# secastel/phaser

Hardware: AMD Instinct MI355X
Metric: het-SNP allele calls/sec + phased variants/sec, whole-genome RNA-seq, 1→8 GPUs (higher is better)
Workload: dtype u8/int32; 1 GPU; configs[2]: whole genome (22 autosomes), one GTEx-shape RNA-seq sample, 79999998 records x 76 bp, 1499988 het SNPs, one shard per chromosome; chromosomes LPT-assigned to GPUs by record count; records=79999998, het_snps=1499988

## Files before the change

### phaser_amd/csrc/phz_map.hip

```cpp
#include "phz_internal.h"
#include "phz_lbound.h"
#include "phz_stagepack.h"
#include <stdlib.h>
#include <string.h>

namespace {

#ifndef PHZ_MAP_WIN
#define PHZ_MAP_WIN 512
#endif
#ifndef PHZ_CIG_X2
#define PHZ_CIG_X2 5
#endif
#ifndef PHZ_CAND_X4
#define PHZ_CAND_X4 3
#endif
constexpr int MAP_WIN = PHZ_MAP_WIN;

constexpr uint32_t OP_M = 0, OP_I = 1, OP_D = 2, OP_N = 3, OP_S = 4, OP_EQ = 7, OP_X = 8, OP_G = 9;

struct MapArgs {
    const int32_t *pos;
    const uint32_t *cigar_off, *cigar, *seq_off;
    const uint8_t *seq2, *qual;
    const uint8_t *bq;
    int64_t n;
    const int32_t *vpos;
    int nv;
    int baseq;
    uint2 *stage;
    uint32_t *side;
    int64_t slots;
    const int32_t *tile_w0;
    int32_t *tile_total;
    int slot_cap;
    int64_t ntiles;
    int dbg;
    bool one;
    const struct ShardDev *shp;
};

struct ShardDev {
    const int32_t *pos;
    const uint32_t *cigar_off, *cigar, *seq_off;
    const uint8_t *seq2, *qual;
    const uint8_t *bq;
    int64_t n;
    const int32_t *vpos;
    int nv, pad;
    int32_t *o_read, *o_var;
    uint8_t *o_code;
    uint32_t *o_aux0, *o_aux1;
    int64_t cap;
};

struct MapBatch {
    const ShardDev *shards;
    const int64_t *tile0;
    int n_shards, baseq;
    uint2 *stage;
    uint32_t *side; int64_t slots;
    int32_t *tile_w0;
    int32_t *tile_total;
    int slot_cap, dbg;
    int64_t ntiles;
    unsigned long long *prof;
    const struct OvfArea *ovf;
};
struct OvfArea { uint32_t *tile_first; unsigned long long *cursor; long long base, cap; };

__device__ __forceinline__ int shard_of(const int64_t *tile0, int n_shards, int64_t T) {
    int lo = 0, hi = n_shards - 1;
    while (lo < hi) {
        const int m = (lo + hi + 1) >> 1;
        if (tile0[m] <= T) lo = m; else hi = m - 1;
    }
    return lo;
}

__device__ __noinline__ int masked_base_escape(const MapArgs &a, uint32_t soff, int x) {
    const uint8_t *qual = a.shp->qual, *seq2 = a.shp->seq2;
    const uint32_t q = qual[(size_t)soff * 4 + x], s = (seq2[(size_t)soff + (x >> 2)] >> (2 * (x & 3))) & 3;
    if ((int)(q & 0x7f) < a.baseq) return 4;
    if (q & 0x80) return s == 0 ? 4 : 5;
    return (int)s;
}

struct VarWin {
    const int32_t *g;
    const int32_t *lds;
    int w0, nv, wlen;
    __device__ __forceinline__ int at(int i) const {
        unsigned d = (unsigned)(i - w0);
        return d < (unsigned)wlen ? lds[d] : g[i];
    }
    __device__ __forceinline__ int lower_bound(int lo, int key) const {
        int hi = nv;
        if (lo >= hi) return hi;
        int step = 1;
        while (lo + step < hi && at(lo + step) < key) { lo += step; step <<= 1; }
        if (lo < hi && at(lo) >= key) return lo;
        int h = lo + step < hi ? lo + step : hi;
        int l = lo + 1;
        while (l < h) {
            int m = (l + h) >> 1;
            if (at(m) < key) l = m + 1; else h = m;
        }
        return l;
    }
};

__device__ __forceinline__ void stage_put(uint2 *stage, uint32_t *side, int64_t slots, int64_t g, uint32_t var, uint32_t a0, uint32_t a1,
                                          uint32_t rec, uint32_t code) {
    const bool w0 = a0 >= 0x10000u, w1 = a1 != 0u;
    stage[g] = make_uint2(var, rec | (code << 10) | ((uint32_t)w1 << 14) | ((uint32_t)w0 << 15) | (w0 ? 0u : a0 << 16));
    if (w0) side[g] = a0;
    if (w1) side[slots + g] = a1;
}

struct CigWin {
    const uint32_t *g;
    const uint32_t *lds;
    uint32_t c_begin, cap;
    __device__ __forceinline__ uint32_t at(uint32_t k) const {
        const uint32_t d = k - c_begin;
        return d < cap ? lds[d] : g[k];
    }
};

#ifndef PHZ_CAND_INS
#define PHZ_CAND_INS 16
#endif
constexpr int CAND_INS = PHZ_CAND_INS;
constexpr uint32_t KEY_HAS_INS = 0x4000u;
struct CandBuf {
    uint32_t *key;
    uint16_t *var;
    uint16_t *x0;
    unsigned long long *ins;
    int *n;
    int *nins;
    int cap, w0;
};
__device__ __forceinline__ void cand_put(const CandBuf &cb, int slot, uint32_t key, int var, uint32_t x0, uint32_t x1) {
    const uint32_t dv = (uint32_t)(var - cb.w0);
    bool wide = dv >= 0xFFFFu || (x0 != 0xFFFFFFFFu && x0 >= 0xFFFFu);
    if (x1 != 0u) {
        const int t = atomicAdd(cb.nins, 1);
        if (t < CAND_INS) cb.ins[t] = ((unsigned long long)(uint32_t)slot << 32) | x1; else wide = true;
        key |= KEY_HAS_INS;
    }
    if (wide) atomicOr(cb.n, 1 << 30);
    cb.key[slot] = key;
    cb.var[slot] = (uint16_t)dv;
    cb.x0[slot] = (uint16_t)(x0 == 0xFFFFFFFFu ? 0xFFFFu : x0);
}
__device__ __forceinline__ uint32_t cand_x0(const CandBuf &cb, int e) { const uint32_t v = cb.x0[e]; return v == 0xFFFFu ? 0xFFFFFFFFu : v; }
__device__ __forceinline__ uint32_t cand_x1(const CandBuf &cb, int e, uint32_t key) {
    if (!(key & KEY_HAS_INS)) return 0u;
    const int m = *cb.nins < CAND_INS ? *cb.nins : CAND_INS;
    for (int t = 0; t < m; t++) { const unsigned long long w = cb.ins[t]; if ((int)(w >> 32) == e) return (uint32_t)w; }
    return 0u;
}

#define PHZ_SEQ_BYTE(a, soff, x) (((a).dbg & 1024) ? (a).qual[(size_t)(soff) * 4 + ((x) | 3)] : (a).seq2[(size_t)(soff) + ((x) >> 2)])
#define PHZ_ONEPLANE(a) ((a).one)
__device__ __forceinline__ int masked_base_two(const MapArgs &a, uint32_t soff, int x) {
    const uint32_t q = a.qual[(size_t)soff * 4 + x], s = (a.seq2[(size_t)soff + (x >> 2)] >> (2 * (x & 3))) & 3;
    if ((int)(q & 0x7f) < a.baseq) return 4;
    if (q & 0x80) return s == 0 ? 4 : 5;
    return (int)s;
}
__device__ int masked_base_escape(const MapArgs &a, uint32_t soff, int x);
__device__ __forceinline__ int sym_from_bq(const MapArgs &a, uint32_t soff, int x, uint32_t b) {
    const uint32_t q6 = b & 63u;
    if (q6 == 63u) return a.qual ? masked_base_two(a, soff, x) : masked_base_escape(a, soff, x);
    return (int)q6 < a.baseq ? 4 : (int)(b >> 6);
}
__device__ __forceinline__ int masked_base(const MapArgs &a, uint32_t soff, int x) {
    if (PHZ_ONEPLANE(a)) return sym_from_bq(a, soff, x, a.bq[(size_t)soff * 4 + x]);
    uint32_t q = a.qual[(size_t)soff * 4 + x];
    uint32_t s = (PHZ_SEQ_BYTE(a, soff, x) >> (2 * (x & 3))) & 3;
    if ((int)(q & 0x7f) < a.baseq) return 4;
    if (q & 0x80) return s == 0 ? 4 : 5;
    return (int)s;
}

template <int MODE, bool NARROW = false>
__device__ int walk_read(const MapArgs &a, const VarWin &vw, const CigWin &cw, const CandBuf &cb, int j, int64_t r, int pos,
                         uint32_t c0, uint32_t c1, uint32_t soff, int64_t out_base, int64_t out_limit) {
    int i = vw.lower_bound(vw.w0, pos);
    if (i >= vw.nv) return 0;
    int cnt = 0;
    int gpos = 0, rpos = 0, seg_start = 0, plen = 0, seg_rpos = 0;
    uint32_t seg_op = c0;
    for (uint32_t k = c0; k < c1; k++) {
        uint32_t w = cw.at(k);
        const int len = (int)(w >> 4);
        const uint32_t op = w & 15;
        if (op == OP_M || op == OP_EQ || op == OP_X || op == OP_D) {
            const int lo = pos + seg_start + plen, hi = lo + len;
            if (i < vw.nv && vw.at(i) < lo) i = vw.lower_bound(i, lo);
            while (i < vw.nv && !(a.dbg & 16)) {
                const int vp = vw.at(i);
                if (vp >= hi) break;
                const int p = vp - pos - seg_start;
                const int rb = rpos + (p - plen);
                int ioff = 0, ilen = 0;
                if (c1 - c0 > 1) {
                    int g2 = seg_start, r2 = seg_rpos;
                    for (uint32_t k2 = seg_op; k2 < c1; k2++) {
                        uint32_t w2 = cw.at(k2);
                        const int l2 = (int)(w2 >> 4);
                        const uint32_t o2 = w2 & 15;
                        if (o2 == OP_N) break;
                        if (o2 == OP_M || o2 == OP_EQ || o2 == OP_X) { g2 += l2; r2 += l2; }
                        else if (o2 == OP_D || o2 == OP_G) g2 += l2;
                        else if (o2 == OP_I) { if (g2 - 1 == p) { ioff = r2; ilen = l2; } r2 += l2; }
                        else if (o2 == OP_S) r2 += l2;
                    }
                }
                const int nchars = (op != OP_D) + ilen;
                if (nchars > 0) {
                    const uint32_t x0 = op != OP_D ? (uint32_t)rb : 0xFFFFFFFFu;
                    const uint32_t x1 = ilen > 0 ? (((uint32_t)ioff << 12) | (uint32_t)(ilen > 4095 ? 4095 : ilen)) : 0u;
                    if (MODE == 0) {
                        const int slot = cnt < 32 ? atomicAdd(cb.n, 1) : (atomicOr(cb.n, 1 << 30), 1 << 30);
                        if (slot < cb.cap) cand_put(cb, slot, ((uint32_t)j << 16) | ((uint32_t)cnt << 8) | (nchars == 1 ? 7u : 4u), i, x0, x1);
                        cnt++;
                    } else {
                        int code = 4;
                        if (nchars == 1) {
                            const int s = masked_base(a, soff, op != OP_D ? rb : ioff);
                            code = s < 4 ? s : (s == 4 ? -1 : 4);
                        }
                        if (code >= 0) {
                            if (MODE == 2) {
                                const int64_t o = out_base + cnt;
                                if (o < out_limit) {
                                    if (NARROW) reinterpret_cast<uint32_t *>(a.stage)[o] = stage4_pack((uint32_t)i, (uint32_t)j, (uint32_t)code);
                                    else stage_put(a.stage, a.side, a.slots, o, (uint32_t)i, x0, x1, (uint32_t)j, (uint32_t)code);
                                }
                            }
                            cnt++;
                        }
                    }
                }
                i++;
            }
            plen += len; gpos += len;
            if (op != OP_D) rpos += len;
        } else if (op == OP_I || op == OP_S) {
            rpos += len;
        } else if (op == OP_N) {
            gpos += len; seg_start = gpos; plen = 0; seg_op = k + 1; seg_rpos = rpos;
        } else if (op == OP_G) {
            gpos += len;
        }
    }
    return cnt;
}

#ifndef PHZ_WIN_DSMALL
#define PHZ_WIN_DSMALL 7
#endif
constexpr int WIN_DMAX = 31 - __builtin_clz((unsigned)MAP_WIN);
constexpr int WIN_DSMALL = WIN_DMAX < PHZ_WIN_DSMALL ? WIN_DMAX : PHZ_WIN_DSMALL;
static_assert(MAP_WIN >= 2 && MAP_WIN <= 1024 && (MAP_WIN & (MAP_WIN - 1)) == 0, "MAP_WIN: a power of two up to 1024");
__device__ __forceinline__ int window_depth(int wlen) {
    return wlen <= (1 << WIN_DSMALL) ? WIN_DSMALL : WIN_DMAX;
}
__device__ __forceinline__ int lds_lower_bound(const int32_t *w, int wdepth, int key) {
    return wdepth == WIN_DSMALL ? window_lower_bound<WIN_DSMALL>(w, key) : window_lower_bound<WIN_DMAX>(w, key);
}

__device__ bool walk_lean(const int32_t *s_vpos, int wlen, int wdepth, int w0, const uint32_t *s_cig, uint32_t c_begin, uint32_t cig_cap,
                          const CandBuf &cb, uint32_t *s_poison, int j, int pos, uint32_t c0, uint32_t c1, long long cover, int dbg) {
    if (c1 - c_begin > cig_cap) return false;
    int g = 0, seg_start = 0, cnt = 0, nins = 0; uint32_t r = 0;
    bool bad = false;
    int t0 = -1, t1 = -1; uint32_t o0 = 0, o1 = 0, l0 = 0, l1 = 0;
    uint32_t prev = 0x10u, prev_len = 1;
    for (uint32_t k = c0; k < c1; k++) {
        const uint32_t w = s_cig[k - c_begin];
        const int len = (int)(w >> 4); const uint32_t op = w & 15, bit = 1u << op;
        const bool mlike = (bit & 0x181u) != 0;
        if (__builtin_amdgcn_uicmp(op, OP_I, 32 ) != 0) {
            if (op == OP_I) {
                bad |= (prev & 0x272u) != 0 || prev_len == 0 || nins == 2;
                nins++;
                t1 = t0; o1 = o0; l1 = l0; t0 = g - 1 + seg_start; o0 = r; l0 = (uint32_t)(len > 4095 ? 4095 : len);
            }
        }
        bad |= op == OP_G;
        const bool search = (mlike || op == OP_D) && !(dbg & 64);
        if (__builtin_amdgcn_ballot_w64(search) != 0) {
            const int lo = pos + g;
            bad |= search && (long long)lo + len > cover;
            const int hi = (search && !bad) ? lo + len : lo;
            int i = lds_lower_bound(s_vpos, wdepth, lo);
            while (i < wlen && !(dbg & 128)) {
                const int vp = s_vpos[i];
                if (vp >= hi) break;
                uint32_t ioff = 0, ilen = 0;
                if (seg_start == 0) {
                    if (vp == hi - 1 && k + 1 < c1) {
                        const uint32_t wn = s_cig[k + 1 - c_begin];
                        if ((wn & 15) == OP_I) { ilen = wn >> 4; ilen = ilen > 4095u ? 4095u : ilen; ioff = r + (mlike ? (uint32_t)len : 0u); }
                    }
                } else {
                    const int off = vp - pos;
                    if (t0 == off) { ioff = o0; ilen = l0; } else if (t1 == off) { ioff = o1; ilen = l1; }
                }
                const int nchars = (mlike ? 1 : 0) + (int)ilen;
                if (nchars > 0) {
                    const int slot = cnt < 32 ? atomicAdd(cb.n, 1) : (atomicOr(cb.n, 1 << 30), 1 << 30);
                    if (slot < cb.cap)
                        cand_put(cb, slot, ((uint32_t)j << 16) | ((uint32_t)(cnt | 0x80) << 8) | (nchars == 1 ? 7u : 4u), w0 + i,
                                 mlike ? (uint32_t)(r + (uint32_t)(vp - lo)) : 0xFFFFFFFFu, ilen > 0 ? ((ioff << 12) | ilen) : 0u);
                    cnt++;
                }
                i++;
            }
        }
        g += len & __builtin_amdgcn_sbfe(0x38D, op, 1u);
        r += (uint32_t)(len & __builtin_amdgcn_sbfe(0x193, op, 1u));
        if (op == OP_N) { seg_start = g; t0 = -1; t1 = -1; }
        prev = bit; prev_len = (uint32_t)len;
    }
    if (bad) atomicOr(&s_poison[j >> 5], 1u << (j & 31));
    return !bad;
}

constexpr int MAP_COVER = 65536;
constexpr int MAP_SLACK = 8;

__global__ void k_tile_window(MapBatch bt, int tile_reads) {
    const int64_t T = (int64_t)blockIdx.x * blockDim.x + threadIdx.x;
    if (T == 0) *bt.ovf->cursor = 0ull;
    const bool live = T < bt.ntiles;
    const int si = live ? shard_of(bt.tile0, bt.n_shards, T) : 0;
    const ShardDev &sh = bt.shards[si];
    const int64_t t = live ? T - bt.tile0[si] : 0;
    const int32_t *pos = sh.pos; const uint32_t *cigar_off = sh.cigar_off; const int32_t *vpos = sh.vpos;
    const int nv = sh.nv; const int64_t n = sh.n;
    int32_t *tile_w = bt.tile_w0;
    const int key = live ? pos[t * tile_reads] : 0;
    const uint32_t coff0 = live ? cigar_off[t * tile_reads] : 0u;
    const int nb_key = __shfl_down(key, 1);
    const uint32_t nb_coff0 = (uint32_t)__shfl_down((int)coff0, 1);
    if (!live) return;
    const bool more = (t + 1) * tile_reads < n;
    const int64_t last = more ? (t + 1) * tile_reads - 1 : n - 1;
    const bool nb = more && (threadIdx.x & 63) != 63;
    const uint32_t coff_end = nb ? nb_coff0 : cigar_off[last + 1];
    const int pos_end = (nb && (long long)nb_key - key <= MAP_COVER) ? nb_key : pos[last];
    const long long key2 = (long long)pos_end + MAP_COVER;
    int lo = 0, hi = nv, lo2 = 0, hi2 = nv;
    while (lo < hi || lo2 < hi2) {
        const int m = (lo + hi) >> 1, m2 = (lo2 + hi2) >> 1;
        const bool go = lo < hi, go2 = lo2 < hi2;
        const int v = go ? vpos[m] : 0, v2 = go2 ? vpos[m2] : 0;
        if (go) { if (v < key) lo = m + 1; else hi = m; }
        if (go2) { if ((long long)v2 < key2) lo2 = m2 + 1; else hi2 = m2; }
    }
    int len = lo2 - lo + MAP_SLACK;
    int complete = 1 << 30;
    if (len > MAP_WIN) { len = MAP_WIN; complete = 0; }
    const uint32_t n_ops = coff_end - coff0;
    tile_w[4 * T] = lo;
    tile_w[4 * T + 1] = len | complete | (si << 16);
    tile_w[4 * T + 2] = (int32_t)coff0;
    tile_w[4 * T + 3] = (int32_t)n_ops;
}

__device__ __forceinline__ int wave_incl_scan(int v0) {
    int v1 = v0 + __builtin_amdgcn_update_dpp(0, v0, 0x111, 0xf, 0xf, true);
    v1 += __builtin_amdgcn_update_dpp(0, v0, 0x112, 0xf, 0xf, true);
    v1 += __builtin_amdgcn_update_dpp(0, v0, 0x113, 0xf, 0xf, true);
    v1 += __builtin_amdgcn_update_dpp(0, v1, 0x114, 0xf, 0xe, true);
    v1 += __builtin_amdgcn_update_dpp(0, v1, 0x118, 0xf, 0xc, true);
    v1 += __builtin_amdgcn_update_dpp(0, v1, 0x142, 0xa, 0xf, true);
    v1 += __builtin_amdgcn_update_dpp(0, v1, 0x143, 0xc, 0xf, true);
    return v1;
}

__device__ __forceinline__ int wave_max(int v0) {
    const int lo = (int)0x80000000;
    auto mx = [](int a, int b) { return a > b ? a : b; };
    int v1 = mx(v0, __builtin_amdgcn_update_dpp(lo, v0, 0x111, 0xf, 0xf, false));
    v1 = mx(v1, __builtin_amdgcn_update_dpp(lo, v0, 0x112, 0xf, 0xf, false));
    v1 = mx(v1, __builtin_amdgcn_update_dpp(lo, v0, 0x113, 0xf, 0xf, false));
    v1 = mx(v1, __builtin_amdgcn_update_dpp(lo, v1, 0x114, 0xf, 0xe, false));
    v1 = mx(v1, __builtin_amdgcn_update_dpp(lo, v1, 0x118, 0xf, 0xc, false));
    v1 = mx(v1, __builtin_amdgcn_update_dpp(lo, v1, 0x142, 0xa, 0xf, false));
    v1 = mx(v1, __builtin_amdgcn_update_dpp(lo, v1, 0x143, 0xc, 0xf, false));
    return __builtin_amdgcn_readlane(v1, 63);
}

template <int MAP_BLOCK, int RPT>
__device__ __forceinline__ int block_scan(const int (&cnt)[RPT], int (&excl)[RPT], int (*s_wsum)[MAP_BLOCK / 64], int lane, int wave) {
    int incl[RPT];
#pragma unroll
    for (int k = 0; k < RPT; k++) {
        const int x = wave_incl_scan(cnt[k]);
        incl[k] = x;
        if (lane == 63) s_wsum[k][wave] = x;
    }
    __syncthreads();
    int running = 0;
#pragma unroll
    for (int k = 0; k < RPT; k++) {
        int before = running;
#pragma unroll
        for (int w2 = 0; w2 < MAP_BLOCK / 64; w2++) {
            const int s = s_wsum[k][w2];
            if (w2 < wave) before += s;
            running += s;
        }
        excl[k] = before + incl[k] - cnt[k];
    }
    return running;
}

template <int MAP_BLOCK, int RPT, bool ABL, bool ONE, bool NARROW>
__device__ __forceinline__ void map_tile(const MapBatch &bt, const int64_t gtile) {
    const int4 tw = *reinterpret_cast<const int4 *>(bt.tile_w0 + 4 * gtile);
    const int si = (tw.y >> 16) & 0x1FFF;
    MapArgs a;
    {
        const ShardDev &sh = bt.shards[si];
        a.pos = sh.pos; a.cigar_off = sh.cigar_off; a.cigar = sh.cigar; a.seq_off = sh.seq_off; a.bq = sh.bq; a.shp = &sh;
        if (ONE && !ABL) { a.seq2 = nullptr; a.qual = nullptr; } else { a.seq2 = sh.seq2; a.qual = sh.qual; }
        a.n = sh.n; a.vpos = sh.vpos; a.nv = sh.nv; a.baseq = bt.baseq;
        a.stage = bt.stage; a.side = bt.side; a.slots = bt.slots;
        a.tile_w0 = bt.tile_w0; a.tile_total = bt.tile_total; a.slot_cap = bt.slot_cap; a.ntiles = bt.ntiles; a.dbg = ABL ? bt.dbg : 0;
        a.one = ABL ? ((bt.dbg & 4096) != 0 && sh.bq != nullptr) : ONE;
    }
#define PHZ_STAMP(K) do { if (ABL && (bt.dbg & 2048) && threadIdx.x == 0) bt.prof[8 * gtile + (K)] = wall_clock64(); } while (0)
    PHZ_STAMP(0);
    constexpr int TILE = MAP_BLOCK * RPT;
    constexpr int CIG = TILE * PHZ_CIG_X2 / 2;
    constexpr int CAND = TILE * PHZ_CAND_X4 / 4;
    __shared__ int32_t s_vpos[MAP_WIN];
    __shared__ uint32_t s_coff[TILE + 1];
    __shared__ uint32_t s_soff[TILE];
    __shared__ int32_t s_pos[TILE];
    uint32_t *s_mask = reinterpret_cast<uint32_t *>(s_pos);
    __shared__ uint16_t s_cx[TILE];
    __shared__ uint32_t s_cig[CIG];
    __shared__ uint32_t s_key[CAND];
    __shared__ uint16_t s_var[CAND];
    __shared__ uint16_t s_x0[CAND];
    __shared__ unsigned long long s_ins[CAND_INS];
    __shared__ int s_wsum[RPT][MAP_BLOCK / 64];
    __shared__ int s_ncand, s_ncx, s_nlong, s_nins;
    __shared__ uint32_t s_poison[TILE / 32];

    const int tid = threadIdx.x, lane = tid & 63, wave = tid >> 6;
    const int64_t tile = gtile - bt.tile0[si];
    const int64_t r0 = tile * TILE;
    const int nr = (int)((a.n - r0) < TILE ? (a.n - r0) : TILE);

    VarWin vw;
    vw.g = a.vpos; vw.lds = s_vpos; vw.nv = a.nv; vw.w0 = tw.x;
    vw.wlen = tw.y & 0xFFFF;
    const bool complete = (tw.y >> 30) & 1;
    CigWin cw;
    cw.g = a.cigar; cw.lds = s_cig; cw.c_begin = (uint32_t)tw.z; cw.cap = CIG;
    uint32_t cnt_w = (uint32_t)tw.w;
    if (cnt_w > (uint32_t)CIG) cnt_w = CIG;
    int rpos_[RPT];
    uint32_t soff_[RPT], coff_[RPT];
#pragma unroll
    for (int k = 0; k < RPT; k++) {
        const int j = k * MAP_BLOCK + tid;
        const bool ok = j < nr;
        rpos_[k] = ok ? a.pos[r0 + j] : 0;
        soff_[k] = ok ? a.seq_off[r0 + j] : 0;
        coff_[k] = a.cigar_off[r0 + (ok ? j : nr)];
    }
    const uint32_t coff_end = a.cigar_off[r0 + nr];
    int v_first = 0x7fffffff;
    if (tid < vw.wlen) { const int idx = vw.w0 + tid; v_first = idx < a.nv ? a.vpos[idx] : 0x7fffffff; }
    uint32_t cg[3] = {0, 0, 0};
#pragma unroll
    for (int u = 0; u < 3; u++) { const uint32_t j = (uint32_t)tid + (uint32_t)u * MAP_BLOCK; if (j < cnt_w) cg[u] = a.cigar[cw.c_begin + j]; }
#pragma unroll
    for (int k = 0; k < RPT; k++) {
        const int j = k * MAP_BLOCK + tid;
        s_pos[j] = rpos_[k]; s_soff[j] = soff_[k]; s_coff[j] = coff_[k];
    }
    if (tid == 0) { s_coff[TILE] = coff_end; s_ncand = 0; s_ncx = 0; s_nlong = 0; s_nins = 0; }
    if (tid < TILE / 32) s_poison[tid] = 0;
    const int wdepth = window_depth(vw.wlen);
#ifdef PHZ_FILL_ALL
    const int wfill = MAP_WIN;
#else
    const int wfill = (1 << wdepth) > vw.wlen ? (1 << wdepth) : vw.wlen;
#endif
    if (tid < wfill) s_vpos[tid] = v_first;
    for (int j = tid + MAP_BLOCK; j < wfill; j += MAP_BLOCK) {
        const int idx = vw.w0 + j;
        s_vpos[j] = (j < vw.wlen && idx < a.nv) ? a.vpos[idx] : 0x7fffffff;
    }
#pragma unroll
    for (int u = 0; u < 3; u++) { const uint32_t j = (uint32_t)tid + (uint32_t)u * MAP_BLOCK; if (j < cnt_w) s_cig[j] = cg[u]; }
    for (uint32_t j = (uint32_t)tid + 3u * MAP_BLOCK; j < cnt_w; j += MAP_BLOCK) s_cig[j] = a.cigar[cw.c_begin + j];
    __syncthreads();
    PHZ_STAMP(1);
    CandBuf cb;
    cb.key = s_key; cb.var = s_var; cb.x0 = s_x0; cb.ins = s_ins; cb.n = &s_ncand; cb.nins = &s_nins; cb.cap = CAND; cb.w0 = vw.w0;
    const long long cover = (long long)s_pos[nr - 1] + MAP_COVER;

    uint32_t c0_[RPT], c1_[RPT];
    int base_[RPT], n_[RPT];
    uint32_t vmask_[RPT], codes_[RPT];
    bool fast_[RPT];
#pragma unroll
    for (int k = 0; k < RPT; k++) {
        const int j = k * MAP_BLOCK + tid;
        c0_[k] = s_coff[j]; c1_[k] = s_coff[j + 1];
        base_[k] = 0; n_[k] = 0; vmask_[k] = 0; codes_[k] = 0; fast_[k] = false;
    }
    const bool walk_on = !(a.dbg & 8);
    int len_[RPT]; bool one_[RPT];
#pragma unroll
    for (int k = 0; k < RPT; k++) {
        const int j = k * MAP_BLOCK + tid;
        one_[k] = false; len_[k] = 0;
        const uint32_t d = c0_[k] - cw.c_begin;
        if (j < nr && walk_on && complete && c1_[k] - c0_[k] == 1 && d < (uint32_t)CIG) {
            const uint32_t w = s_cig[d];
            const uint32_t op = w & 15;
            len_[k] = (int)(w >> 4);
            one_[k] = (op == OP_M || op == OP_EQ || op == OP_X) && (long long)rpos_[k] + len_[k] <= cover;
        }
    }
    constexpr int GROUP = 64 / (2 * RPT);
    int target = 0x7fffffff;
#pragma unroll
    for (int k = 0; k < RPT; k++) {
        const int e = wave_max(one_[k] ? rpos_[k] + len_[k] : (int)0x80000000);
        const int first = __builtin_amdgcn_readfirstlane(rpos_[k]);
        if ((lane / GROUP) == 2 * k) target = first;
        if ((lane / GROUP) == 2 * k + 1) target = e;
    }
    const int bound = lds_lower_bound(s_vpos, wdepth, target);
#pragma unroll
    for (int k = 0; k < RPT; k++) {
        const int j = k * MAP_BLOCK + tid;
        const int lo = __builtin_amdgcn_readlane(bound, 2 * k * GROUP), hi = __builtin_amdgcn_readlane(bound, (2 * k + 1) * GROUP);
        if (one_[k]) {
            const int pos = rpos_[k], end = pos + len_[k];
            if (hi - lo <= 24) {
                int below = 0, c = 0;
                for (int e = lo; e < hi; e++) {
                    const int vp = s_vpos[e];
                    below += vp < pos ? 1 : 0;
                    c += (vp >= pos && vp < end) ? 1 : 0;
                }
                if (c <= 8) { fast_[k] = true; base_[k] = lo + below; n_[k] = c; }
            } else {
                const int base = lds_lower_bound(s_vpos, wdepth, pos);
                int c = 0;
                while (base + c < vw.wlen && s_vpos[base + c] < end && c <= 8) c++;
                if (c <= 8) { fast_[k] = true; base_[k] = base; n_[k] = c; }
            }
        }
        if (j < nr && walk_on && !fast_[k]) {
            if (s_coff[j + 1] - s_coff[j] > 3u) s_cx[TILE - 1 - atomicAdd(&s_nlong, 1)] = (uint16_t)j;
            else s_cx[atomicAdd(&s_ncx, 1)] = (uint16_t)j;
        }
    }
    uint32_t pre_q[RPT], pre_s[RPT];
#pragma unroll
    for (int k = 0; k < RPT; k++) {
        pre_q[k] = 0; pre_s[k] = 0;
        if (fast_[k] && n_[k] > 0 && !(a.dbg & 1)) {
            const uint32_t soff = s_soff[k * MAP_BLOCK + tid];
            const int x = s_vpos[base_[k]] - rpos_[k];
            if (PHZ_ONEPLANE(a)) pre_q[k] = a.bq[(size_t)soff * 4 + x];
            else { pre_q[k] = a.qual[(size_t)soff * 4 + x]; pre_s[k] = PHZ_SEQ_BYTE(a, soff, x); }
        }
    }
    PHZ_STAMP(2);
    __syncthreads();
    PHZ_STAMP(3);
    const int nshort = walk_on ? s_ncx : 0;
    const int ncx = (walk_on && !(a.dbg & 256)) ? nshort + s_nlong : 0;
    const bool lean_on = complete && !(a.dbg & 32);
    bool redo_any = false;
    for (int t = tid; t < ncx; t += MAP_BLOCK) {
        const int ts = t < nshort ? t : TILE - 1 - (t - nshort);
        const int j = s_cx[ts];
        const bool done = lean_on && walk_lean(s_vpos, vw.wlen, wdepth, vw.w0, s_cig, cw.c_begin, (uint32_t)CIG, cb, s_poison, j, s_pos[j], s_coff[j], s_coff[j + 1], cover, a.dbg);
        if (!done) { s_cx[ts] = (uint16_t)(j | 0x8000); redo_any = true; }
    }
    const bool redo = __syncthreads_or(redo_any ? 1 : 0) != 0;
#pragma unroll
    for (int k = 0; k < RPT; k++) s_mask[k * MAP_BLOCK + tid] = 0;
    if (redo) {
        for (int t = tid; t < ncx; t += MAP_BLOCK) {
            const int jf = s_cx[t < nshort ? t : TILE - 1 - (t - nshort)];
            if (jf & 0x8000) { const int j = jf & 0x7FFF; walk_read<0>(a, vw, cw, cb, j, r0 + j, a.pos[r0 + j], s_coff[j], s_coff[j + 1], 0, 0, 0); }
        }
    }
    __syncthreads();
    PHZ_STAMP(4);
    const int ncand = s_ncand;
    const bool fb = ncand > CAND;
    uint32_t cq = 0, cs = 0; int cx_off = -1;
    if (!fb && tid < ncand && !(a.dbg & 1)) {
        const uint32_t key = s_key[tid];
        if ((key & 0xFF) == 7u) {
            const uint32_t x0 = cand_x0(cb, tid);
            cx_off = x0 != 0xFFFFFFFFu ? (int)x0 : (int)(cand_x1(cb, tid, key) >> 12);
            const uint32_t soff = s_soff[key >> 16];
            if (PHZ_ONEPLANE(a)) cq = a.bq[(size_t)soff * 4 + cx_off];
            else { cq = a.qual[(size_t)soff * 4 + cx_off]; cs = PHZ_SEQ_BYTE(a, soff, cx_off); }
        }
    }
#pragma unroll
    for (int k = 0; k < RPT; k++) {
        if (!fast_[k]) continue;
        const int j = k * MAP_BLOCK + tid;
        const uint32_t soff = s_soff[j];
        for (int o = 0; o < n_[k]; o++) {
            const int x = s_vpos[base_[k] + o] - rpos_[k];
            int sy;
            if (a.dbg & 1) sy = x & 3;
            else if (o == 0) {
                if (PHZ_ONEPLANE(a)) sy = sym_from_bq(a, soff, x, pre_q[k]);
                else {
                    const uint32_t q = pre_q[k], sb = (pre_s[k] >> (2 * (x & 3))) & 3;
                    sy = (int)(q & 0x7f) < a.baseq ? 4 : ((q & 0x80) ? (sb == 0 ? 4 : 5) : (int)sb);
                }
            } else sy = masked_base(a, soff, x);
            if (sy != 4) { vmask_[k] |= 1u << o; codes_[k] |= (uint32_t)(sy < 4 ? sy : 4) << (4 * o); }
        }
    }
    int cnt[RPT], off[RPT];
    if (!fb) {
        for (int e = tid; e < ncand; e += MAP_BLOCK) {
            uint32_t key = s_key[e];
            const int j = (int)(key >> 16);
            int code = (int)(key & 0xFF);
            if ((key & 0x8000u) && ((s_poison[j >> 5] >> (j & 31)) & 1u)) code = -1;
            else if (code == 7) {
                const uint32_t x0 = cand_x0(cb, e);
                const int x = x0 != 0xFFFFFFFFu ? (int)x0 : (int)(cand_x1(cb, e, key) >> 12);
                int sy;
                if (a.dbg & 1) sy = x & 3;
                else if (e == tid && cx_off == x) {
                    if (PHZ_ONEPLANE(a)) sy = sym_from_bq(a, s_soff[j], x, cq);
                    else {
                        const uint32_t sb = (cs >> (2 * (x & 3))) & 3;
                        sy = (int)(cq & 0x7f) < a.baseq ? 4 : ((cq & 0x80) ? (sb == 0 ? 4 : 5) : (int)sb);
                    }
                } else sy = masked_base(a, s_soff[j], x);
                code = sy < 4 ? sy : (sy == 4 ? -1 : 4);
            }
            if (code >= 0) {
                atomicOr(&s_mask[j], 1u << ((key >> 8) & 31));
                s_key[e] = (key & 0xFFFFFF00u) | (uint32_t)code;
            } else {
                s_key[e] = key | 0xFFu;
            }
        }
        __syncthreads();
#pragma unroll
        for (int k = 0; k < RPT; k++) cnt[k] = fast_[k] ? __popc(vmask_[k]) : __popc(s_mask[k * MAP_BLOCK + tid]);
    } else {
#pragma unroll
        for (int k = 0; k < RPT; k++) {
            const int j = k * MAP_BLOCK + tid;
            cnt[k] = fast_[k] ? __popc(vmask_[k])
                              : (j < nr && walk_on ? walk_read<1>(a, vw, cw, cb, j, r0 + j, NARROW ? a.pos[r0 + j] : rpos_[k], NARROW ? s_coff[j] : c0_[k],
                                                                  NARROW ? s_coff[j + 1] : c1_[k], s_soff[j], 0, 0) : 0);
        }
    }
    PHZ_STAMP(5);
    const int T = block_scan<MAP_BLOCK, RPT>(cnt, off, s_wsum, lane, wave);
#pragma unroll
    for (int k = 0; k < RPT; k++) s_coff[k * MAP_BLOCK + tid] = (uint32_t)off[k];
    if (tid == 0) {
        a.tile_total[gtile] = T;
        uint32_t first = (uint32_t)(gtile * (int64_t)a.slot_cap);
        int room = a.slot_cap;
        if (T > a.slot_cap) {
            const OvfArea ov = *bt.ovf;
            const unsigned long long at = atomicAdd(ov.cursor, (unsigned long long)T);
            const bool fits = at + (unsigned long long)T <= (unsigned long long)ov.cap;
            if (fits) { first = (uint32_t)(ov.base + (long long)at); room = T; }
            ov.tile_first[gtile] = fits ? first : 0xFFFFFFFFu;
        }
        s_ncx = (int)first; s_nlong = room;
    }
    __syncthreads();
    PHZ_STAMP(6);
    if (a.dbg & 2) return;
    const int64_t slot0 = (int64_t)(uint32_t)s_ncx;
    const int slot_n = s_nlong;
#pragma unroll
    for (int k = 0; k < RPT; k++) {
        const int j = k * MAP_BLOCK + tid;
        if (fast_[k]) {
            int o2 = off[k];
            for (int o = 0; o < n_[k]; o++) {
                if (!((vmask_[k] >> o) & 1)) continue;
                if (o2 < slot_n) {
                    const int64_t g = slot0 + o2;
                    if (NARROW) reinterpret_cast<uint32_t *>(a.stage)[g] = stage4_pack((uint32_t)(vw.w0 + base_[k] + o), (uint32_t)j, (codes_[k] >> (4 * o)) & 15u);
                    else stage_put(a.stage, a.side, a.slots, g, (uint32_t)(vw.w0 + base_[k] + o), (uint32_t)(s_vpos[base_[k] + o] - rpos_[k]), 0u,
                                   (uint32_t)j, (codes_[k] >> (4 * o)) & 15u);
                }
                o2++;
            }
        } else if (fb && cnt[k] > 0) {
            walk_read<2, NARROW>(a, vw, cw, cb, j, r0 + j, NARROW ? a.pos[r0 + j] : rpos_[k], NARROW ? a.cigar_off[r0 + j] : c0_[k],
                                 NARROW ? a.cigar_off[r0 + j + 1] : c1_[k], s_soff[j], slot0 + off[k], slot0 + slot_n);
        }
    }
    if (!fb) {
        for (int e = tid; e < ncand; e += MAP_BLOCK) {
            const uint32_t key = s_key[e];
            if ((key & 0xFF) == 0xFF) continue;
            const int j = (int)(key >> 16);
            const uint32_t ord = (key >> 8) & 31;
            const int o = (int)s_coff[j] + __popc(s_mask[j] & ((1u << ord) - 1));
            if (o < slot_n) {
                const int64_t g = slot0 + o;
                if (NARROW) reinterpret_cast<uint32_t *>(a.stage)[g] = stage4_pack((uint32_t)(vw.w0 + (int)s_var[e]), (uint32_t)j, key & 15u);
                else stage_put(a.stage, a.side, a.slots, g, (uint32_t)(vw.w0 + (int)s_var[e]), cand_x0(cb, e), cand_x1(cb, e, key), (uint32_t)j, key & 15u);
            }
        }
    }
    PHZ_STAMP(7);
#undef PHZ_STAMP
}

#ifndef PHZ_MAP_WAVES
#define PHZ_MAP_WAVES 8
#endif
#if PHZ_MAP_WAVES > 0
#define PHZ_MAP_OCC __attribute__((amdgpu_waves_per_eu(PHZ_MAP_WAVES, PHZ_MAP_WAVES)))
#else
#define PHZ_MAP_OCC
#endif
template <int MAP_BLOCK, int RPT, bool ABL, bool ONE = false, bool NARROW = false>
__global__ __launch_bounds__(MAP_BLOCK) PHZ_MAP_OCC void k_map(MapBatch bt) {
    map_tile<MAP_BLOCK, RPT, ABL, ONE, NARROW>(bt, (int64_t)blockIdx.x);
}

__global__ __launch_bounds__(1024) void k_chunk_scan(const int32_t *tile_total, int64_t ntiles, int32_t *tile_pref, int64_t *chunk_sum,
                                                     int32_t *chunk_max) {
    __shared__ int s_w[16], s_m[16];
    const int tid = threadIdx.x, lane = tid & 63, wave = tid >> 6;
    const int64_t i = (int64_t)blockIdx.x * 1024 + tid;
    const int v = i < ntiles ? tile_total[i] : 0;
    int x = v, mx = v;
#pragma unroll
    for (int d = 1; d < 64; d <<= 1) {
        int y = __shfl_up(x, d);
        if (lane >= d) x += y;
    }
#pragma unroll
    for (int d = 32; d >= 1; d >>= 1) { int y = __shfl_xor(mx, d); mx = y > mx ? y : mx; }
    if (lane == 63) s_w[wave] = x;
    if (lane == 0) s_m[wave] = mx;
    __syncthreads();
    int before = 0;
    for (int w2 = 0; w2 < wave; w2++) before += s_w[w2];
    if (i < ntiles) tile_pref[i] = before + x - v;
    if (tid == 1023) chunk_sum[blockIdx.x] = before + x;
    if (tid == 0) {
        int m = 0;
        for (int w2 = 0; w2 < 16; w2++) m = s_m[w2] > m ? s_m[w2] : m;
        chunk_max[blockIdx.x] = m;
    }
}

__device__ __forceinline__ int64_t calls_before(const int64_t *chunk_base, const int32_t *tile_pref, int64_t T) {
    return chunk_base[T >> 10] + tile_pref[T];
}

struct TotalsOut {
    const int64_t *tile0; int n_shards; int64_t ntiles;
    const int32_t *tile_pref;
    int64_t *shard_base;
    const unsigned long long *cursor;
    unsigned long long *host;
};
__device__ __forceinline__ void shard_total(const TotalsOut &o, int s, const int64_t *chunk_base, int64_t total) {
    const int64_t a = o.tile0[s], b = o.tile0[s + 1];
    const int64_t lo = a < o.ntiles ? calls_before(chunk_base, o.tile_pref, a) : total;
    const int64_t hi = b < o.ntiles ? calls_before(chunk_base, o.tile_pref, b) : total;
    o.shard_base[s] = lo;
    o.host[2 + s] = (unsigned long long)(hi - lo);
}
__device__ __forceinline__ void batch_words(const TotalsOut &o, unsigned long long total, unsigned long long max_tile) {
    o.host[0] = total; o.host[1] = max_tile; o.host[2 + o.n_shards] = *o.cursor;
}

constexpr int BASE_LDS = 1024;
__global__ __launch_bounds__(1024) void k_chunk_base(const int64_t *chunk_sum, const int32_t *chunk_max, int nchunks, int64_t *chunk_base,
                                                     unsigned long long *scal, bool merged, TotalsOut o) {
    __shared__ long long s_w[16];
    __shared__ long long s_carry;
    __shared__ int s_m[16];
    __shared__ int64_t s_base[BASE_LDS];
    const int tid = threadIdx.x, lane = tid & 63, wave = tid >> 6;
    if (tid == 0) s_carry = 0;
    int mx = 0;
    __syncthreads();
    for (int b0 = 0; b0 < nchunks; b0 += 1024) {
        const int i = b0 + tid;
        const long long v = i < nchunks ? chunk_sum[i] : 0;
        if (i < nchunks) mx = chunk_max[i] > mx ? chunk_max[i] : mx;
        long long x = v;
#pragma unroll
        for (int d = 1; d < 64; d <<= 1) {
            long long y = __shfl_up(x, d);
            if (lane >= d) x += y;
        }
        if (lane == 63) s_w[wave] = x;
        __syncthreads();
        long long before = s_carry;
        for (int w2 = 0; w2 < wave; w2++) before += s_w[w2];
        if (i < nchunks) { chunk_base[i] = before + x - v; if (merged) s_base[i] = before + x - v; }
        __syncthreads();
        if (tid == 1023) s_carry = before + x;
        __syncthreads();
    }
#pragma unroll
    for (int d = 32; d >= 1; d >>= 1) { int y = __shfl_xor(mx, d); mx = y > mx ? y : mx; }
    if (lane == 0) s_m[wave] = mx;
    __syncthreads();
    const long long total = s_carry;
    if (tid == 0) {
        int m = 0;
        for (int w2 = 0; w2 < 16; w2++) m = s_m[w2] > m ? s_m[w2] : m;
        scal[0] = (unsigned long long)total;
        scal[1] = (unsigned long long)m;
        if (merged) batch_words(o, (unsigned long long)total, (unsigned long long)m);
    }
    if (merged)
        for (int s = tid; s < o.n_shards; s += 1024) shard_total(o, s, s_base, total);
}

__global__ void k_shard_totals(const int64_t *chunk_base, const unsigned long long *scal, TotalsOut o) {
    const int s = blockIdx.x * blockDim.x + threadIdx.x;
    if (s == 0) batch_words(o, scal[0], scal[1]);
    if (s < o.n_shards) shard_total(o, s, chunk_base, (int64_t)scal[0]);
}

struct CompactArgs {
    const uint2 *stage; const uint32_t *side; int64_t slots;
    const ShardDev *shards; const int64_t *tile0; int n_shards;
    const int32_t *tile_total; const int32_t *tile_pref; const int64_t *chunk_base; const int64_t *shard_base;
    const int32_t *tile_w0;
    int slot_cap, tile_reads; int64_t ntiles;
    const uint32_t *tile_ovf;
};

#ifndef PHZ_CT
#define PHZ_CT 4
#endif
constexpr int CT = PHZ_CT, CT_UNR = 4;
struct ShardOut { int32_t *o_read, *o_var; uint8_t *o_code; uint32_t *o_aux0, *o_aux1; int64_t cap; };
__device__ __forceinline__ ShardOut shard_out(const ShardDev &sh) { return ShardOut{sh.o_read, sh.o_var, sh.o_code, sh.o_aux0, sh.o_aux1, sh.cap}; }

template <bool UNI, bool AUX, bool NARROW>
__device__ __forceinline__ void compact_run(const CompactArgs &c, const int *pref, const int64_t *dstv, const int32_t *r0v, const int32_t *siv, const int64_t *slotv,
                                            int M, int lane, const ShardOut &out0) {
    static_assert(!(AUX && NARROW), "the narrow staging word carries no text planes");
    if (NARROW) {
        const uint32_t *stage4 = reinterpret_cast<const uint32_t *>(c.stage);
        for (int e0 = lane; e0 < M; e0 += 64 * CT_UNR) {
            int k_[CT_UNR]; uint32_t w_[CT_UNR];
#pragma unroll
            for (int u = 0; u < CT_UNR; u++) {
                const int e = e0 + 64 * u;
                int k = 0;
#pragma unroll
                for (int st = CT / 2; st > 0; st >>= 1) k += (pref[k + st] <= e) ? st : 0;
                k_[u] = k;
                w_[u] = e < M ? stage4[slotv[k] + (e - pref[k])] : 0u;
            }
#pragma unroll
            for (int u = 0; u < CT_UNR; u++) {
                const int e = e0 + 64 * u;
                if (e >= M) break;
                const int k = k_[u];
                const uint32_t w = w_[u];
                const ShardOut sh = UNI ? out0 : shard_out(c.shards[siv[k]]);
                const int64_t o = dstv[k] + (e - pref[k]);
                if (o < sh.cap) {
                    sh.o_read[o] = r0v[k] + (int32_t)stage4_rec(w);
                    sh.o_var[o] = (int32_t)stage4_var(w);
                    sh.o_code[o] = (uint8_t)stage4_code(w);
                }
// ... 312 lines not shown
```

Measured before the change: 16.73 billion allele calls/s.

## Make lean CIGAR walk branch-free and wave-uniform with templated window depth

Moves the per-read lean CIGAR walk into a shared header. Each op step now uses sbfe table masks and a wave-ballot loop bound, with neutral ops padding shorter reads, so lanes stay converged. The window lower-bound depth becomes a template parameter picked once per tile, and the per-thread strided loop becomes an unrolled RPT loop. The small-window fast path counts variants as below_end minus below, removing the per-element range test. The cost is extra iterations of neutral ops for short reads in a wave, plus more code from template instantiation.

```diff
diff --git a/phaser_amd/csrc/phz_leanwalk.h b/phaser_amd/csrc/phz_leanwalk.h
--- /dev/null
+++ b/phaser_amd/csrc/phz_leanwalk.h
@@ -0,0 +1,87 @@
+#pragma once
+#include <stdint.h>
+
+#if defined(__HIPCC__) || defined(__CUDACC__)
+#define PHZ_LW_FN __device__ __forceinline__
+#else
+#define PHZ_LW_FN inline
+#endif
+
+PHZ_LW_FN uint32_t lean_mask(uint32_t table, uint32_t op) {
+#if defined(__HIP_DEVICE_COMPILE__)
+    return (uint32_t)__builtin_amdgcn_sbfe((int)table, op, 1u);
+#else
+    return 0u - ((table >> op) & 1u);
+#endif
+}
+
+constexpr uint32_t LEAN_OP_I = 1, LEAN_OP_N = 3;
+constexpr uint32_t LEAN_T_MLIKE = 0x181u;
+constexpr uint32_t LEAN_T_SEARCH = 0x185u;
+constexpr uint32_t LEAN_T_REF = 0x38Du;
+constexpr uint32_t LEAN_T_READ = 0x193u;
+constexpr uint32_t LEAN_T_NOINS = 0x272u;
+constexpr uint32_t LEAN_T_G = 0x200u;
+constexpr uint32_t LEAN_NEUTRAL = 6u;
+constexpr uint32_t LEAN_INS_MAX = 4095u;
+
+struct LeanWalk {
+    int g;
+    uint32_t r;
+    int seg_start;
+    int cnt;
+    uint32_t nins;
+    int t0, t1;
+    uint32_t x0, x1;
+    uint32_t prev, prev_len;
+    uint32_t bad;
+};
+
+PHZ_LW_FN void lean_init(LeanWalk &s) {
+    s.g = 0; s.r = 0; s.seg_start = 0; s.cnt = 0; s.nins = 0; s.t0 = -1; s.t1 = -1; s.x0 = 0; s.x1 = 0;
+    s.prev = 0x10u; s.prev_len = 1; s.bad = 0;
+}
+
+struct LeanOp {
+    int lo, hi;
+    uint32_t mlike;
+    uint32_t rbase;
+    uint32_t rnext;
+    uint32_t search;
+};
+
+PHZ_LW_FN LeanOp lean_step(LeanWalk &s, uint32_t w, int pos, long long cover) {
+    const int len = (int)(w >> 4); const uint32_t op = w & 15u, bit = 1u << op;
+    LeanOp o;
+    o.mlike = lean_mask(LEAN_T_MLIKE, op);
+    o.search = lean_mask(LEAN_T_SEARCH, op);
+    if (op == LEAN_OP_I) {
+        s.bad |= (s.prev & LEAN_T_NOINS) | (uint32_t)(s.prev_len == 0) | (uint32_t)(s.nins == 2);
+        s.nins++;
+        const uint32_t l = (uint32_t)len > LEAN_INS_MAX ? LEAN_INS_MAX : (uint32_t)len;
+        s.t1 = s.t0; s.x1 = s.x0; s.t0 = s.g - 1 + s.seg_start; s.x0 = (s.r << 12) | l;
+    }
+    s.bad |= bit & LEAN_T_G;
+    o.lo = pos + s.g;
+    s.bad |= o.search & (uint32_t)((long long)o.lo + len > cover);
+    o.hi = o.lo + (s.bad == 0 ? (len & (int)o.search) : 0);
+    o.rbase = s.r;
+    s.g += len & (int)lean_mask(LEAN_T_REF, op);
+    s.r += (uint32_t)len & lean_mask(LEAN_T_READ, op);
+    o.rnext = s.r;
+    if (op == LEAN_OP_N) { s.seg_start = s.g; s.t0 = -1; s.t1 = -1; }
+    s.prev = bit; s.prev_len = (uint32_t)len;
+    return o;
+}
+
+PHZ_LW_FN uint32_t lean_ins_ahead(const LeanOp &o, int vp, uint32_t wnext) {
+    if (vp != o.hi - 1 || (wnext & 15u) != LEAN_OP_I) return 0u;
+    const uint32_t l = (wnext >> 4) > LEAN_INS_MAX ? LEAN_INS_MAX : (wnext >> 4);
+    return l ? ((o.rnext << 12) | l) : 0u;
+}
+
+PHZ_LW_FN uint32_t lean_ins_carried(const LeanWalk &s, int vp, int pos) {
+    const int off = vp - pos;
+    const uint32_t x = s.t0 == off ? s.x0 : (s.t1 == off ? s.x1 : 0u);
+    return (x & LEAN_INS_MAX) ? x : 0u;
+}
diff --git a/phaser_amd/csrc/phz_map.hip b/phaser_amd/csrc/phz_map.hip
--- a/phaser_amd/csrc/phz_map.hip
+++ b/phaser_amd/csrc/phz_map.hip
@@ -1,5 +1,6 @@
 #include "phz_internal.h"
 #include "phz_lbound.h"
+#include "phz_leanwalk.h"
 #include "phz_stagepack.h"
 #include <stdlib.h>
 #include <string.h>
@@ -274,62 +275,60 @@
     return wdepth == WIN_DSMALL ? window_lower_bound<WIN_DSMALL>(w, key) : window_lower_bound<WIN_DMAX>(w, key);
 }
 
-__device__ bool walk_lean(const int32_t *s_vpos, int wlen, int wdepth, int w0, const uint32_t *s_cig, uint32_t c_begin, uint32_t cig_cap,
+template <int D>
+__device__ bool walk_lean(const int32_t *s_vpos, int wlen, int w0, const uint32_t *s_cig, uint32_t c_begin, uint32_t cig_cap,
                           const CandBuf &cb, uint32_t *s_poison, int j, int pos, uint32_t c0, uint32_t c1, long long cover, int dbg) {
     if (c1 - c_begin > cig_cap) return false;
-    int g = 0, seg_start = 0, cnt = 0, nins = 0; uint32_t r = 0;
-    bool bad = false;
-    int t0 = -1, t1 = -1; uint32_t o0 = 0, o1 = 0, l0 = 0, l1 = 0;
-    uint32_t prev = 0x10u, prev_len = 1;
-    for (uint32_t k = c0; k < c1; k++) {
-        const uint32_t w = s_cig[k - c_begin];
-        const int len = (int)(w >> 4); const uint32_t op = w & 15, bit = 1u << op;
-        const bool mlike = (bit & 0x181u) != 0;
-        if (__builtin_amdgcn_uicmp(op, OP_I, 32 ) != 0) {
-            if (op == OP_I) {
-                bad |= (prev & 0x272u) != 0 || prev_len == 0 || nins == 2;
-                nins++;
-                t1 = t0; o1 = o0; l1 = l0; t0 = g - 1 + seg_start; o0 = r; l0 = (uint32_t)(len > 4095 ? 4095 : len);
+    LeanWalk s; lean_init(s);
+    const uint32_t nops = c1 - c0;
+    const uint32_t *cig = s_cig + (c0 - c_begin);
+    for (uint32_t u = 0; __builtin_amdgcn_ballot_w64(u < nops) != 0; u++) {
+        const uint32_t w = u < nops ? cig[u] : LEAN_NEUTRAL;
+        LeanOp o = lean_step(s, w, pos, (dbg & 64) ? 0x7fffffffffffffffll : cover);
+        if (dbg & 64) { o.search = 0; o.hi = o.lo; }
+        if (__builtin_amdgcn_ballot_w64(o.search != 0) != 0) {
+            int i = window_lower_bound<D>(s_vpos, o.lo);
+            int vp = s_vpos[i & (MAP_WIN - 1)];
+            bool hit = i < wlen && vp < o.hi && !(dbg & 128);
+            if (__builtin_amdgcn_ballot_w64(hit) != 0) {
+                while (hit) {
+                    const uint32_t x1 = s.seg_start == 0 ? lean_ins_ahead(o, vp, u + 1 < nops ? cig[u + 1] : LEAN_NEUTRAL) : lean_ins_carried(s, vp, pos);
+                    const int nchars = (int)(o.mlike & 1u) + (int)(x1 & LEAN_INS_MAX);
+                    if (nchars > 0) {
+                        const int slot = s.cnt < 32 ? atomicAdd(cb.n, 1) : (atomicOr(cb.n, 1 << 30), 1 << 30);
+                        if (slot < cb.cap)
+                            cand_put(cb, slot, ((uint32_t)j << 16) | ((uint32_t)(s.cnt | 0x80) << 8) | (nchars == 1 ? 7u : 4u), w0 + i,
+                                     o.mlike ? o.rbase + (uint32_t)(vp - o.lo) : 0xFFFFFFFFu, x1);
+                        s.cnt++;
+                    }
+                    i++;
+                    vp = s_vpos[i & (MAP_WIN - 1)];
+                    hit = i < wlen && vp < o.hi;
+                }
             }
         }
-        bad |= op == OP_G;
-        const bool search = (mlike || op == OP_D) && !(dbg & 64);
-        if (__builtin_amdgcn_ballot_w64(search) != 0) {
-            const int lo = pos + g;
-            bad |= search && (long long)lo + len > cover;
-            const int hi = (search && !bad) ? lo + len : lo;
-            int i = lds_lower_bound(s_vpos, wdepth, lo);
-            while (i < wlen && !(dbg & 128)) {
-                const int vp = s_vpos[i];
-                if (vp >= hi) break;
-                uint32_t ioff = 0, ilen = 0;
-                if (seg_start == 0) {
-                    if (vp == hi - 1 && k + 1 < c1) {
-                        const uint32_t wn = s_cig[k + 1 - c_begin];
-                        if ((wn & 15) == OP_I) { ilen = wn >> 4; ilen = ilen > 4095u ? 4095u : ilen; ioff = r + (mlike ? (uint32_t)len : 0u); }
-                    }
-                } else {
-                    const int off = vp - pos;
-                    if (t0 == off) { ioff = o0; ilen = l0; } else if (t1 == off) { ioff = o1; ilen = l1; }
-                }
-                const int nchars = (mlike ? 1 : 0) + (int)ilen;
-                if (nchars > 0) {
-                    const int slot = cnt < 32 ? atomicAdd(cb.n, 1) : (atomicOr(cb.n, 1 << 30), 1 << 30);
-                    if (slot < cb.cap)
-                        cand_put(cb, slot, ((uint32_t)j << 16) | ((uint32_t)(cnt | 0x80) << 8) | (nchars == 1 ? 7u : 4u), w0 + i,
-                                 mlike ? (uint32_t)(r + (uint32_t)(vp - lo)) : 0xFFFFFFFFu, ilen > 0 ? ((ioff << 12) | ilen) : 0u);
-                    cnt++;
-                }
-                i++;
-            }
-        }
-        g += len & __builtin_amdgcn_sbfe(0x38D, op, 1u);
-        r += (uint32_t)(len & __builtin_amdgcn_sbfe(0x193, op, 1u));
-        if (op == OP_N) { seg_start = g; t0 = -1; t1 = -1; }
-        prev = bit; prev_len = (uint32_t)len;
-    }
-    if (bad) atomicOr(&s_poison[j >> 5], 1u << (j & 31));
-    return !bad;
+    }
+    if (s.bad) atomicOr(&s_poison[j >> 5], 1u << (j & 31));
+    return s.bad == 0;
+}
+
+template <int D, int MAP_BLOCK, int RPT>
+__device__ __forceinline__ uint32_t lean_pass(bool lean_on, int tid, int ncx, int nshort, uint16_t *s_cx, const int32_t *s_vpos, int wlen, int w0,
+                                              const uint32_t *s_cig, uint32_t c_begin, const CandBuf &cb, uint32_t *s_poison, const int32_t *s_pos,
+                                              const uint32_t *s_coff, long long cover, int dbg) {
+    constexpr int TILE = MAP_BLOCK * RPT;
+    uint32_t redo_any = 0;
+#pragma unroll
+    for (int k = 0; k < RPT; k++) {
+        const int t = k * MAP_BLOCK + tid;
+        if (t < ncx) {
+            const int ts = t < nshort ? t : TILE - 1 - (t - nshort);
+            const int j = s_cx[ts];
+            const bool done = lean_on && walk_lean<D>(s_vpos, wlen, w0, s_cig, c_begin, (uint32_t)(TILE * PHZ_CIG_X2 / 2), cb, s_poison, j, s_pos[j], s_coff[j], s_coff[j + 1], cover, dbg);
+            if (!done) { s_cx[ts] = (uint16_t)(j | 0x8000); redo_any = 1u; }
+        }
+    }
+    return redo_any;
 }
 
 constexpr int MAP_COVER = 65536;
@@ -551,17 +550,18 @@
     for (int k = 0; k < RPT; k++) {
         const int j = k * MAP_BLOCK + tid;
         const int lo = __builtin_amdgcn_readlane(bound, 2 * k * GROUP), hi = __builtin_amdgcn_readlane(bound, (2 * k + 1) * GROUP);
-        if (one_[k]) {
-            const int pos = rpos_[k], end = pos + len_[k];
+        {
+            const int pos = rpos_[k], end = (int)((uint32_t)pos + (uint32_t)len_[k]);
             if (hi - lo <= 24) {
-                int below = 0, c = 0;
+                int below = 0, below_end = 0;
                 for (int e = lo; e < hi; e++) {
                     const int vp = s_vpos[e];
                     below += vp < pos ? 1 : 0;
-                    c += (vp >= pos && vp < end) ? 1 : 0;
+                    below_end += vp < end ? 1 : 0;
                 }
-                if (c <= 8) { fast_[k] = true; base_[k] = lo + below; n_[k] = c; }
-            } else {
+                const int c = below_end - below;
+                if (one_[k] && c <= 8) { fast_[k] = true; base_[k] = lo + below; n_[k] = c; }
+            } else if (one_[k]) {
                 const int base = lds_lower_bound(s_vpos, wdepth, pos);
                 int c = 0;
                 while (base + c < vw.wlen && s_vpos[base + c] < end && c <= 8) c++;
@@ -590,14 +590,10 @@
     const int nshort = walk_on ? s_ncx : 0;
     const int ncx = (walk_on && !(a.dbg & 256)) ? nshort + s_nlong : 0;
     const bool lean_on = complete && !(a.dbg & 32);
-    bool redo_any = false;
-    for (int t = tid; t < ncx; t += MAP_BLOCK) {
-        const int ts = t < nshort ? t : TILE - 1 - (t - nshort);
-        const int j = s_cx[ts];
-        const bool done = lean_on && walk_lean(s_vpos, vw.wlen, wdepth, vw.w0, s_cig, cw.c_begin, (uint32_t)CIG, cb, s_poison, j, s_pos[j], s_coff[j], s_coff[j + 1], cover, a.dbg);
-        if (!done) { s_cx[ts] = (uint16_t)(j | 0x8000); redo_any = true; }
-    }
-    const bool redo = __syncthreads_or(redo_any ? 1 : 0) != 0;
+    const uint32_t redo_any = wdepth == WIN_DSMALL
+        ? lean_pass<WIN_DSMALL, MAP_BLOCK, RPT>(lean_on, tid, ncx, nshort, s_cx, s_vpos, vw.wlen, vw.w0, s_cig, cw.c_begin, cb, s_poison, s_pos, s_coff, cover, a.dbg)
+        : lean_pass<WIN_DMAX, MAP_BLOCK, RPT>(lean_on, tid, ncx, nshort, s_cx, s_vpos, vw.wlen, vw.w0, s_cig, cw.c_begin, cb, s_poison, s_pos, s_coff, cover, a.dbg);
+    const bool redo = __syncthreads_or((int)redo_any) != 0;
 #pragma unroll
     for (int k = 0; k < RPT; k++) s_mask[k * MAP_BLOCK + tid] = 0;
     if (redo) {
```

Measured after the change: 17.49 billion allele calls/s (median of 6 runs). 4.5% higher.
